# zabaras/deep-turbulence

Measured on AMD Instinct MI355X. Metric: flow-field samples/sec (fwd+log-det+bwd), 64x256x256x4; optimizer step: HipAdam (one-launch Adam, same update as torch.optim.Adam), higher is better.
Workload: dtype f32

## Files before the change

deep-turbulence_amd/csrc/tmg_common.h:

```cpp
#pragma once
#include <hip/hip_runtime.h>
#include <stdint.h>
#include <stdlib.h>
#include <atomic>

typedef float f32x4 __attribute__((ext_vector_type(4)));

__device__ __forceinline__ __amdgpu_buffer_rsrc_t tmg_make_rsrc(const void* base, unsigned bytes) {
    return __builtin_amdgcn_make_buffer_rsrc(const_cast<void*>(base), 0, (int)bytes, 0x00020000);
}
__device__ __forceinline__ float4 tmg_bload4(__amdgpu_buffer_rsrc_t rs, unsigned voff, unsigned soff) {
    const f32x4 v = __builtin_bit_cast(f32x4, __builtin_amdgcn_raw_buffer_load_b128(rs, (int)voff, (int)soff, 0));
    return make_float4(v[0], v[1], v[2], v[3]);
}

#define TMG_MAX_IN_SEG 3
#define TMG_MAX_OUT_SEG 3

struct TmgSeg {
    const float* p;
    int stride;
    int off;
    int n;
};
// ... 1 lines not shown
    float* p;
    int stride;
    int off;
    int n;
};

__device__ __forceinline__ float wave_sum(float v) {
#pragma unroll
    for (int o = 32; o > 0; o >>= 1) v += __shfl_xor(v, o, 64);
    return v;
}

__device__ __forceinline__ float block_sum_256(float v, float* red ) {
    v = wave_sum(v);
    const int lane = threadIdx.x & 63, w = threadIdx.x >> 6;
    __syncthreads();
    if (lane == 0) red[w] = v;
    __syncthreads();
    return red[0] + red[1] + red[2] + red[3];
}

__device__ __forceinline__ float out_scale_of(const float* kappa) {
    if (!kappa) return 1.0f;
    float k = *kappa;
    k = fminf(fmaxf(k, -4.0f), 1.3862943611198906f);
    return expf(k);
}

#define TMG_PICK_SEG(PTYPE_, ARR, C_, PTR_, STRIDE_, OFF_)                                                \
    PTYPE_ PTR_ = ARR[0].p;                                                                               \
    int STRIDE_ = ARR[0].stride, OFF_ = ARR[0].off;                                                       \
    if (C_ >= ARR[0].n) {                                                                                 \
        C_ -= ARR[0].n; PTR_ = ARR[1].p; STRIDE_ = ARR[1].stride; OFF_ = ARR[1].off;                      \
        if (C_ >= ARR[1].n) { C_ -= ARR[1].n; PTR_ = ARR[2].p; STRIDE_ = ARR[2].stride; OFF_ = ARR[2].off; } \
    }
#define TMG_PICK_OSEG(ARR, NL_, PTR_, STRIDE_, OFF_) TMG_PICK_SEG(float*, ARR, NL_, PTR_, STRIDE_, OFF_)

template <typename P>
__device__ __forceinline__ float4 load_in4(const P& p, int b, int iy, int ix, int c) {
    float4 v = make_float4(0.f, 0.f, 0.f, 0.f);
    if (p.pad_rep) {
        iy = min(max(iy, 0), p.Hin - 1);
        ix = min(max(ix, 0), p.Win - 1);
    } else if (iy < 0 || iy >= p.Hin || ix < 0 || ix >= p.Win) {
        return v;
    }
    if (c >= p.Cin) return v;
    const size_t pix = ((size_t)b * p.Hin + iy) * p.Win + ix;
    if (p.vec4) {
        int cl = c;
        TMG_PICK_SEG(const float*, p.in, cl, sp, ss, so)
        v = *reinterpret_cast<const float4*>(sp + pix * ss + so + cl);
    } else {
        float t[4];
#pragma unroll
        for (int e = 0; e < 4; ++e) {
            int cl = c + e;
            float x = 0.f;
            if (cl < p.Cin) {
                TMG_PICK_SEG(const float*, p.in, cl, sp, ss, so)
                x = sp[pix * ss + so + cl];
            }
            t[e] = x;
        }
        v = make_float4(t[0], t[1], t[2], t[3]);
    }
    if (p.in_scale) {
        float* f = reinterpret_cast<float*>(&v);
#pragma unroll
        for (int e = 0; e < 4; ++e)
            if (c + e < p.Cin) f[e] = f[e] * p.in_scale[c + e] + p.in_shift[c + e];
    }
    if (p.relu_in) {
        v.x = fmaxf(v.x, 0.f);
        v.y = fmaxf(v.y, 0.f);
        v.z = fmaxf(v.z, 0.f);
        v.w = fmaxf(v.w, 0.f);
    }
    return v;
}

template <int U = 8, typename P>
__device__ __forceinline__ void stage_patch(const P& p, float* lds, int b, int iy0, int ix0, int PH, int PW, int c0,
                                            int kch, int CS, int swz = 0) {
    const int k4 = kch >> 2;
    const int items = PH * PW * k4;
    const int nt = blockDim.x;
    const unsigned mk = k4 > 1 ? 0xFFFFFFFFu / (unsigned)k4 + 1u : 0u;
    const unsigned mp = 0xFFFFFFFFu / (unsigned)PW + 1u;
    for (int base = threadIdx.x; base < items; base += nt * U) {
        float4 v[U];
        int dst[U];
#pragma unroll
        for (int u = 0; u < U; ++u) {
            const int it = base + u * nt;
            dst[u] = -1;
            if (it < items) {
                const int pix = k4 > 1 ? (int)__umulhi((unsigned)it, mk) : it;
                const int c4 = it - pix * k4;
                const int py = (int)__umulhi((unsigned)pix, mp);
                const int px = pix - py * PW;
                v[u] = load_in4(p, b, iy0 + py, ix0 + px, c0 + 4 * c4);
                dst[u] = pix * CS + ((4 * c4) ^ ((px & 1) ? swz : 0));
            }
        }
#pragma unroll
        for (int u = 0; u < U; ++u)
            if (dst[u] >= 0) *reinterpret_cast<float4*>(lds + dst[u]) = v[u];
    }
}

static __device__ float tmg_zero_page[64];

#if defined(__HIP_DEVICE_COMPILE__)
#define TMG_PACKED_F32 __attribute__((target("packed-fp32-ops")))
#else
#define TMG_PACKED_F32
#endif

typedef float f32x2 __attribute__((ext_vector_type(2)));
#define TMG_GAS __attribute__((address_space(1)))
__device__ __forceinline__ float4 tmg_ldg4(const float* p) {
    const f32x4 v = *(const TMG_GAS f32x4*)p;
    return make_float4(v[0], v[1], v[2], v[3]);
}
__device__ __forceinline__ float2 tmg_ldg2(const float* p) {
    const f32x2 v = *(const TMG_GAS f32x2*)p;
    return make_float2(v[0], v[1]);
}
__device__ __forceinline__ float tmg_ldg1(const float* p) { return *(const TMG_GAS float*)p; }

__device__ __forceinline__ int tmg_xcd_block(int b, int G) {
    if (G < 16) return b;
    const int qn = G >> 3, rn = G & 7, x = b & 7;
    return x * qn + min(x, rn) + (b >> 3);
}
struct TmgTileRange { int first, end, step; };
__device__ __forceinline__ TmgTileRange tmg_xcd_tiles(int ntiles, int b, int G) {
    if (G < 16 || ntiles < 64) return TmgTileRange{b, ntiles, G};
    const int x = b & 7;
    const int nb = (G >> 3) + (x < (G & 7) ? 1 : 0);
    const int lo = (int)(((long long)ntiles * x) >> 3), hi = (int)(((long long)ntiles * (x + 1)) >> 3);
    return TmgTileRange{lo + (b >> 3), hi, nb};
}

template <typename P>
__device__ __forceinline__ const float* in4_addr(const P& p, int b, int iy, int ix, int c, bool& oob) {
    const int iyc = min(max(iy, 0), p.Hin - 1), ixc = min(max(ix, 0), p.Win - 1);
    oob = !p.pad_rep && (iy != iyc || ix != ixc);
    const size_t pix = ((size_t)b * p.Hin + iyc) * p.Win + ixc;
    int cl = c;
    TMG_PICK_SEG(const float*, p.in, cl, sp, ss, so)
    const float* a = sp + pix * ss + so + cl;
    return (oob || c >= p.Cin) ? tmg_zero_page : a;
}

template <int U = 4, typename P>
__device__ __forceinline__ void stage_patch_bf(const P& p, float* lds, int b, int iy0, int ix0, int PH, int PW, int c0,
                                               int kch, int CS) {
    if (!p.vec4) {
        stage_patch<U>(p, lds, b, iy0, ix0, PH, PW, c0, kch, CS);
        return;
    }
    const int k4 = kch >> 2;
    const int items = PH * PW * k4;
    const int nt = blockDim.x;
    const unsigned mk = k4 > 1 ? 0xFFFFFFFFu / (unsigned)k4 + 1u : 0u;
    const unsigned mp = 0xFFFFFFFFu / (unsigned)PW + 1u;
    for (int base = threadIdx.x; base < items; base += nt * U) {
        float4 v[U];
        const float* a[U];
        int dst[U];
        unsigned oobm = 0;
#pragma unroll
        for (int u = 0; u < U; ++u) {
            const int it = min(base + u * nt, items - 1);
            const int pix = k4 > 1 ? (int)__umulhi((unsigned)it, mk) : it;
            const int c4 = it - pix * k4;
            const int py = (int)__umulhi((unsigned)pix, mp);
            const int px = pix - py * PW;
            bool oob;
            a[u] = in4_addr(p, b, iy0 + py, ix0 + px, c0 + 4 * c4, oob);
            oobm |= (oob ? 1u : 0u) << u;
            dst[u] = (base + u * nt < items) ? pix * CS + 4 * c4 : -1;
        }
#pragma unroll
        for (int u = 0; u < U; ++u) v[u] = *reinterpret_cast<const float4*>(a[u]);
#pragma unroll
        for (int u = 0; u < U; ++u) {
            if (p.in_scale && !((oobm >> u) & 1u)) {
                const int it = min(base + u * nt, items - 1);
                const int pix = k4 > 1 ? (int)__umulhi((unsigned)it, mk) : it;
                const int c = c0 + 4 * (it - pix * k4);
                float* f = reinterpret_cast<float*>(&v[u]);
#pragma unroll
                for (int e = 0; e < 4; ++e)
                    if (c + e < p.Cin) f[e] = f[e] * p.in_scale[c + e] + p.in_shift[c + e];
            }
            if (p.relu_in) {
                v[u].x = fmaxf(v[u].x, 0.f); v[u].y = fmaxf(v[u].y, 0.f);
                v[u].z = fmaxf(v[u].z, 0.f); v[u].w = fmaxf(v[u].w, 0.f);
            }
            if (dst[u] >= 0) *reinterpret_cast<float4*>(lds + dst[u]) = v[u];
        }
    }
}

template <int U>
struct StageRegs {
    float4 v[U];
    int dst[U];
};

template <int U, typename P>
__device__ __forceinline__ void stage_issue(const P& p, StageRegs<U>& R, int b, int iy0, int ix0, int PH, int PW, int c0, int kch,
                                            int CS) {
    const int k4 = kch >> 2;
    const int items = PH * PW * k4;
    const int nt = blockDim.x;
    const unsigned mk = k4 > 1 ? 0xFFFFFFFFu / (unsigned)k4 + 1u : 0u;
    const unsigned mp = 0xFFFFFFFFu / (unsigned)PW + 1u;
#pragma unroll
    for (int u = 0; u < U; ++u) {
        const int it = threadIdx.x + u * nt;
        R.dst[u] = -1;
        if (it < items) {
            const int pix = k4 > 1 ? (int)__umulhi((unsigned)it, mk) : it;
            const int c4 = it - pix * k4;
            const int py = (int)__umulhi((unsigned)pix, mp);
            const int px = pix - py * PW;
            R.v[u] = load_in4(p, b, iy0 + py, ix0 + px, c0 + 4 * c4);
            R.dst[u] = pix * CS + 4 * c4;
        }
    }
}

template <int U, typename P>
__device__ __forceinline__ void stage_commit(const P& p, StageRegs<U>& R, float* lds, int b, int iy0, int ix0, int PH, int PW,
                                             int c0, int kch, int CS) {
#pragma unroll
    for (int u = 0; u < U; ++u)
        if (R.dst[u] >= 0) *reinterpret_cast<float4*>(lds + R.dst[u]) = R.v[u];
    const int k4 = kch >> 2;
    const int items = PH * PW * k4;
    const unsigned mk = k4 > 1 ? 0xFFFFFFFFu / (unsigned)k4 + 1u : 0u;
    const unsigned mp = 0xFFFFFFFFu / (unsigned)PW + 1u;
    for (int it = threadIdx.x + U * blockDim.x; it < items; it += blockDim.x) {
        const int pix = k4 > 1 ? (int)__umulhi((unsigned)it, mk) : it;
        const int c4 = it - pix * k4;
        const int py = (int)__umulhi((unsigned)pix, mp);
        const int px = pix - py * PW;
        *reinterpret_cast<float4*>(lds + pix * CS + 4 * c4) = load_in4(p, b, iy0 + py, ix0 + px, c0 + 4 * c4);
    }
}

static inline void tmg_lds_optin(const void* fn, std::atomic<uint64_t>& done) {
    int dev = 0;
    (void)hipGetDevice(&dev);
    const uint64_t bit = 1ull << (dev & 63);
    if (done.load(std::memory_order_relaxed) & bit) return;
    (void)hipFuncSetAttribute(fn, hipFuncAttributeMaxDynamicSharedMemorySize, 160 * 1024);
    done.fetch_or(bit, std::memory_order_relaxed);
}
#define TMG_LDS_OPTIN(FN)                                              \
    do {                                                               \
        static std::atomic<uint64_t> done__{0};                        \
        tmg_lds_optin(reinterpret_cast<const void*>(FN), done__);      \
// ... 62 lines not shown
```

deep-turbulence_amd/csrc/tmg_pointwise.hip:

```cpp
#include "tmg_common.h"
#include <stdlib.h>

#define LN5 1.6094379124341003f
#define LOG2PI 1.8378770664093453f

static inline int grid_for(size_t n, int cap = 4096) {
    size_t b = (n + 255) / 256;
    return (int)(b < (size_t)cap ? (b ? b : 1) : cap);
}

__global__ __launch_bounds__(256) void affine_apply_kernel(const float* __restrict__ hh, int hs, int ho, const float* x2, int xs,
                                                           int xo, float* y2, int ys, int yo, float* __restrict__ rsave,
                                                           float* __restrict__ logdet, int pix_per_img, int Ch, int reverse, int vec,
                                                           const float* x1, int x1s, float* y1, int y1s, int hpair) {
    __shared__ float red[4];
    const int b = blockIdx.y;
    const size_t base = (size_t)b * pix_per_img;
    const size_t total = (size_t)pix_per_img * Ch;
    float ld = 0.f;
    if (vec) {
        const int c4n = Ch >> 2;
        const size_t tot4 = (size_t)pix_per_img * c4n;
        for (size_t i = blockIdx.x * (size_t)256 + threadIdx.x; i < tot4; i += (size_t)gridDim.x * 256) {
            const size_t pix = base + i / c4n;
// ... 574 lines not shown
}

__global__ void bn_finalize_kernel(const float* __restrict__ sum, const float* __restrict__ csq, const float* __restrict__ gamma,
                                   const float* __restrict__ beta, float* __restrict__ rmean, float* __restrict__ rvar,
                                   float* __restrict__ out, int C, float n, float eps, float momentum) {
    const int c = blockIdx.x * blockDim.x + threadIdx.x;
    if (c >= C) return;
    const float mean = sum[c] / n, var = csq[c] / n;
    const float rstd = rsqrtf(var + eps);
    const float a = gamma[c] * rstd;
    out[c] = mean;
    out[C + c] = var;
    out[2 * C + c] = rstd;
    out[3 * C + c] = a;
    out[4 * C + c] = beta[c] - mean * a;
    if (rmean) {
        rmean[c] = rmean[c] * (1.f - momentum) + momentum * mean;
        rvar[c] = rvar[c] * (1.f - momentum) + momentum * var * (n / fmaxf(n - 1.f, 1.f));
    }
}

__global__ void bn_bwd_apply_kernel(const float* __restrict__ x, int xs, int xo, const float* __restrict__ g, int gs, int go,
                                    const float* __restrict__ a, const float* __restrict__ bsh, const float* __restrict__ mean,
                                    const float* __restrict__ rstd, const float* __restrict__ gamma, const float* __restrict__ m0,
                                    const float* __restrict__ m1, float* __restrict__ dx, int ds, int dof, size_t npix, int C,
                                    int accumulate, float m_scale) {
    const size_t total = npix * C;
    for (size_t i = blockIdx.x * (size_t)blockDim.x + threadIdx.x; i < total; i += (size_t)gridDim.x * blockDim.x) {
        const size_t pix = i / C;
        const int c = i % C;
        const float xv = x[pix * xs + xo + c];
        const float u = xv * a[c] + bsh[c];
        const float du = u > 0.f ? g[pix * gs + go + c] : 0.f;
        const float xh = (xv - mean[c]) * rstd[c];
        const float v = gamma[c] * rstd[c] * (du - m0[c] * m_scale - xh * m1[c] * m_scale);
        float* d = dx + pix * ds + dof + c;
        *d = accumulate ? (*d + v) : v;
    }
}

__global__ void masked_add_kernel(const float* __restrict__ src, int ss, int so, const float* __restrict__ ref, int rs_, int ro,
                                  const float* __restrict__ add, int as, int ao, float* dst, int ds, int dof, size_t npix, int n,
                                  int accumulate) {
    const size_t total = npix * n;
    for (size_t i = blockIdx.x * (size_t)blockDim.x + threadIdx.x; i < total; i += (size_t)gridDim.x * blockDim.x) {
        const size_t pix = i / n;
        const int c = i % n;
        float v = src ? src[pix * ss + so + c] : 0.f;
        if (ref && !(ref[pix * rs_ + ro + c] > 0.f)) v = 0.f;
        if (add) v += add[pix * as + ao + c];
        float* d = dst + pix * ds + dof + c;
        *d = accumulate ? (*d + v) : v;
    }
}

__global__ __launch_bounds__(256) void masked_add4_kernel(const float* __restrict__ src, int ss, int so, const float* __restrict__ ref, int rs_, int ro,
                                   const float* __restrict__ add, int as, int ao, float* dst, int ds, int dof, unsigned npix, int nq,
                                   int accumulate) {
    const unsigned total = npix * (unsigned)nq;
    for (unsigned i = blockIdx.x * blockDim.x + threadIdx.x; i < total; i += gridDim.x * blockDim.x) {
        const unsigned pix = i / (unsigned)nq;
        const unsigned c = 4u * (i - pix * (unsigned)nq);
        float4 v = src ? *reinterpret_cast<const float4*>(src + (size_t)pix * ss + so + c) : make_float4(0.f, 0.f, 0.f, 0.f);
        if (ref) {
            const float4 r = *reinterpret_cast<const float4*>(ref + (size_t)pix * rs_ + ro + c);
            if (!(r.x > 0.f)) v.x = 0.f;
            if (!(r.y > 0.f)) v.y = 0.f;
            if (!(r.z > 0.f)) v.z = 0.f;
            if (!(r.w > 0.f)) v.w = 0.f;
        }
        if (add) {
            const float4 a = *reinterpret_cast<const float4*>(add + (size_t)pix * as + ao + c);
            v.x += a.x; v.y += a.y; v.z += a.z; v.w += a.w;
        }
        float4* d = reinterpret_cast<float4*>(dst + (size_t)pix * ds + dof + c);
        if (accumulate) {
            const float4 o = *d;
            v.x += o.x; v.y += o.y; v.z += o.z; v.w += o.w;
        }
        *d = v;
    }
}

struct C1P {
    TmgSeg in[TMG_MAX_IN_SEG];
    int nseg, vec4;
    int B, Hin, Win;
    int Cin;
    const float* in_scale;
    const float* in_shift;
    int relu_in, pad_rep;
    const float* w;
    int w_rows, w_split, w_gap;
    const float* add; int add_stride, add_off;
    int fill4;
    float* out; int out_stride, out_off;
    int TW_log2, tiles_x, tiles_y, KCH;
};

__global__ __launch_bounds__(256) void c1_fwd_kernel(C1P p) {
    extern __shared__ __attribute__((aligned(16))) float lds[];
    const int tid = threadIdx.x;
    int t = blockIdx.x;
    const int tx = t % p.tiles_x;
    t /= p.tiles_x;
    const int ty = t % p.tiles_y;
    const int b = t / p.tiles_y;
    const int TWl = p.TW_log2, TW = 1 << TWl, TH = 256 >> TWl;
    const int PW = TW + 2, PH = TH + 2;
    const int oy0 = ty * TH, ox0 = tx * TW;
    const int row = tid >> TWl, col = tid & (TW - 1);
    const int Cpad = (p.Cin + 3) & ~3;
    float acc = 0.f;
    for (int c0 = 0; c0 < Cpad; c0 += p.KCH) {
        const int kch = min(p.KCH, Cpad - c0);
        const int CS = kch + 4;
        float* lw = lds + PH * PW * CS;
        __syncthreads();
        stage_patch_bf(p, lds, b, oy0 - 1, ox0 - 1, PH, PW, c0, kch, CS);
        for (int i = tid; i < 9 * kch; i += 256) {
            const int tap = i / kch, c = i - tap * kch;
            const int cs = c0 + c;
            lw[i] = (cs < p.w_rows) ? p.w[(size_t)(cs + (cs < p.w_split ? 0 : p.w_gap)) * 9 + tap] : 0.f;
        }
        __syncthreads();
#pragma unroll
        for (int tap = 0; tap < 9; ++tap) {
            const int tyy = tap / 3, txx = tap - tyy * 3;
            const float* pp = lds + ((row + tyy) * PW + col + txx) * CS;
            const float* wp = lw + tap * kch;
            for (int c = 0; c < kch; c += 4) {
                const float4 a = *reinterpret_cast<const float4*>(pp + c);
                const float4 w4 = *reinterpret_cast<const float4*>(wp + c);
                acc += a.x * w4.x + a.y * w4.y + a.z * w4.z + a.w * w4.w;
            }
        }
    }
    const int oy = oy0 + row, ox = ox0 + col;
    if (oy < p.Hin && ox < p.Win) {
        const size_t opx = ((size_t)b * p.Hin + oy) * p.Win + ox;
        if (p.add) acc += p.add[opx * p.add_stride + p.add_off];
        float* o = p.out + opx * p.out_stride + p.out_off;
        if (p.fill4) *reinterpret_cast<float4*>(o) = make_float4(acc, 0.f, 0.f, 0.f);
        else *o = acc;
    }
}

struct C1X2P {
    TmgSeg in[TMG_MAX_IN_SEG];
    int nseg, vec4;
    int B, Hin, Win;
    int Cin;
    const float* in_scale;
    const float* in_shift;
    int relu_in, pad_rep;
    const float* w1;
    const float* w2;
    int w_rows, w_split, w_gap, w2_d1;
    const float* add1; int a1_stride, a1_off;
    const float* add2; int a2_stride, a2_off;
    float* out; int out_stride;
    int TW_log2, tiles_x, tiles_y, KCH;
};

template <int CG>
__global__ __launch_bounds__(256) void c1x2_fwd_kernel(C1X2P p) {
    extern __shared__ __attribute__((aligned(16))) float lds[];
    constexpr int NPX = 256 / CG;
    const int tid = threadIdx.x;
    const int pid = tid / CG, cg = tid % CG;
    const bool lead = cg == 0;
    int t = tmg_xcd_block((int)blockIdx.x, (int)gridDim.x);
    const int tx = t % p.tiles_x;
    t /= p.tiles_x;
    const int ty = t % p.tiles_y;
    const int b = t / p.tiles_y;
    const int TWl = p.TW_log2, TW = 1 << TWl, TH = NPX >> TWl;
    const int PW = TW + 4, PH = TH + 4;
    const int RW = TW + 2, RH = TH + 2;
    const int oy0 = ty * TH, ox0 = tx * TW;
    const int row = pid >> TWl, col = pid & (TW - 1);
    const int Cpad = (p.Cin + 3) & ~3;
    int ry[2], rx[2];
    bool rok[2];
    ry[0] = row + 1; rx[0] = col + 1; rok[0] = true;
    const int nring = 2 * RW + 2 * (RH - 2);
    {
        rok[1] = pid < nring;
        int i = rok[1] ? pid : 0;
        if (i < RW) { ry[1] = 0; rx[1] = i; }
        else if (i < 2 * RW) { ry[1] = RH - 1; rx[1] = i - RW; }
        else if (i < 2 * RW + RH - 2) { ry[1] = 1 + i - 2 * RW; rx[1] = 0; }
        else { ry[1] = 1 + i - (2 * RW + RH - 2); rx[1] = RW - 1; }
    }
    const bool ring_wave = (tid & ~63) / CG < nring;
    const int oy = oy0 + row, ox = ox0 + col;
    const bool own = oy < p.Hin && ox < p.Win;
    const size_t opx = ((size_t)b * p.Hin + min(oy, p.Hin - 1)) * p.Win + min(ox, p.Win - 1);
    const float a2v = *((p.add2 && own && lead) ? p.add2 + opx * p.a2_stride + p.a2_off : tmg_zero_page);
    float a1v[2];
    bool rin[2];
#pragma unroll
    for (int u = 0; u < 2; ++u) {
        const int y = oy0 - 1 + ry[u], x = ox0 - 1 + rx[u];
        rin[u] = rok[u] && y >= 0 && y < p.Hin && x >= 0 && x < p.Win;
        const size_t px = ((size_t)b * p.Hin + min(max(y, 0), p.Hin - 1)) * p.Win + min(max(x, 0), p.Win - 1);
        a1v[u] = *((p.add1 && rin[u] && lead) ? p.add1 + px * p.a1_stride + p.a1_off : tmg_zero_page);
    }
    float acc1[2] = {0.f, 0.f}, acc2 = 0.f;
    for (int c0 = 0; c0 < Cpad; c0 += p.KCH) {
        const int kch = min(p.KCH, Cpad - c0);
        const int CS = kch + 4;
        float* lw1 = lds + PH * PW * CS;
        float* lw2 = lw1 + 9 * p.KCH;
        __syncthreads();
        stage_patch_bf(p, lds, b, oy0 - 2, ox0 - 2, PH, PW, c0, kch, CS);
        for (int i = tid; i < 9 * kch; i += 256) {
            const int tap = i / kch, c = i - tap * kch;
            const int cs = c0 + c;
            const bool ok = cs < p.w_rows;
            const size_t r = (size_t)(cs + (cs < p.w_split ? 0 : p.w_gap)) * 9 + tap;
            lw1[i] = ok ? p.w1[r] : 0.f;
            lw2[i] = ok ? p.w2[r] : 0.f;
        }
        __syncthreads();
#pragma unroll
        for (int tap = 0; tap < 9; ++tap) {
            const int tyy = tap / 3, txx = tap - tyy * 3;
            const float* w1p = lw1 + tap * kch;
            const float* w2p = lw2 + tap * kch;
            const float* p0 = lds + ((ry[0] + tyy) * PW + rx[0] + txx) * CS;
            const float* p1 = lds + ((ry[1] + tyy) * PW + rx[1] + txx) * CS;
            for (int c = 4 * cg; c < kch; c += 4 * CG) {
                const float4 wa = *reinterpret_cast<const float4*>(w1p + c);
                const float4 wb = *reinterpret_cast<const float4*>(w2p + c);
                const float4 x0 = *reinterpret_cast<const float4*>(p0 + c);
                acc1[0] += x0.x * wa.x + x0.y * wa.y + x0.z * wa.z + x0.w * wa.w;
                acc2 += x0.x * wb.x + x0.y * wb.y + x0.z * wb.z + x0.w * wb.w;
                if (ring_wave) {
                    const float4 x1 = *reinterpret_cast<const float4*>(p1 + c);
                    acc1[1] += x1.x * wa.x + x1.y * wa.y + x1.z * wa.z + x1.w * wa.w;
                }
            }
        }
    }
#pragma unroll
    for (int o = 1; o < CG; o <<= 1) {
        acc1[0] += __shfl_xor(acc1[0], o);
        acc1[1] += __shfl_xor(acc1[1], o);
        acc2 += __shfl_xor(acc2, o);
    }
    __syncthreads();
    float* ld1 = lds;
    if (lead) {
#pragma unroll
        for (int u = 0; u < 2; ++u)
            if (rok[u]) ld1[ry[u] * RW + rx[u]] = rin[u] ? fmaxf(acc1[u] + a1v[u], 0.f) : 0.f;
    }
    const float d1own = acc1[0] + a1v[0];
    __syncthreads();
    if (!lead) return;
    float w2d[9];
#pragma unroll
    for (int tap = 0; tap < 9; ++tap) w2d[tap] = p.w2[(size_t)p.w2_d1 * 9 + tap];
#pragma unroll
    for (int tap = 0; tap < 9; ++tap) {
        const int tyy = tap / 3, txx = tap - tyy * 3;
        acc2 += w2d[tap] * ld1[(row + tyy) * RW + col + txx];
    }
    if (own) *reinterpret_cast<float4*>(p.out + opx * p.out_stride) = make_float4(d1own, acc2 + a2v, 0.f, 0.f);
}

struct C1BP {
    TmgSeg in[TMG_MAX_IN_SEG];
    int nseg, vec4;
    int B, Hin, Win;
    int Cin;
    const float* in_scale;
    const float* in_shift;
    int relu_in, pad_rep;
    const float* w;
    float* dW;
    const float* dd; int dd_stride, dd_off;
    const float* dref; int dref_stride, dref_off;
    TmgOSeg g[TMG_MAX_OUT_SEG];
    int TW_log2, tiles_x, tiles_y, ntiles, KCH;
};

__global__ __launch_bounds__(256) void c1_bwd_kernel(C1BP p) {
    extern __shared__ __attribute__((aligned(16))) float lds[];
    const int tid = threadIdx.x;
    const int TWl = p.TW_log2, TW = 1 << TWl, TH = 256 >> TWl;
    const int PW = TW + 2, PH = TH + 2;
    const int row = tid >> TWl, col = tid & (TW - 1);
    const int Cpad = (p.Cin + 3) & ~3;
    const int nchunks = (Cpad + p.KCH - 1) / p.KCH;
    float* ldd = lds;
    float* lw = ldd + ((PH * PW + 3) & ~3);
    float* lin = lw + 9 * p.KCH;
    float wacc[2][8];
#pragma unroll
    for (int k = 0; k < 2; ++k)
#pragma unroll
        for (int c = 0; c < 8; ++c) wacc[k][c] = 0.f;

    for (int tile = blockIdx.x; tile < p.ntiles; tile += gridDim.x) {
        int t = tile;
        const int tx = t % p.tiles_x;
        t /= p.tiles_x;
        const int ty = t % p.tiles_y;
        const int b = t / p.tiles_y;
        const int oy0 = ty * TH, ox0 = tx * TW;
        __syncthreads();
        for (int i = tid; i < PH * PW; i += 256) {
            const int py = i / PW, px = i - py * PW;
            const int y = oy0 - 1 + py, x = ox0 - 1 + px;
            float v = 0.f;
            if (y >= 0 && y < p.Hin && x >= 0 && x < p.Win) {
                const size_t pix = ((size_t)b * p.Hin + y) * p.Win + x;
                v = p.dd[pix * p.dd_stride + p.dd_off];
                if (p.dref && !(p.dref[pix * p.dref_stride + p.dref_off] > 0.f)) v = 0.f;
            }
            ldd[i] = v;
        }
        __syncthreads();
        float dnb[9];
#pragma unroll
        for (int tap = 0; tap < 9; ++tap) {
            const int ky = tap / 3, kx = tap - ky * 3;
            dnb[tap] = ldd[(row + 2 - ky) * PW + col + 2 - kx];
        }
        const int oy = oy0 + row, ox = ox0 + col;
        const bool inside = oy < p.Hin && ox < p.Win;
        const size_t opix = ((size_t)b * p.Hin + oy) * p.Win + ox;
#pragma unroll
        for (int ch = 0; ch < 8; ++ch) {
            if (ch >= nchunks) break;
            const int c0 = ch * p.KCH;
            const int kch = min(p.KCH, Cpad - c0);
            const int CS = kch + 4;
            __syncthreads();
            stage_patch_bf(p, lin, b, oy0 - 1, ox0 - 1, PH, PW, c0, kch, CS);
            for (int i = tid; i < 9 * kch; i += 256) {
                const int tap = i / kch, c = i - tap * kch;
                lw[i] = (c0 + c < p.Cin) ? p.w[(size_t)(c0 + c) * 9 + tap] : 0.f;
            }
            __syncthreads();
            if (inside) {
                for (int c = 0; c < kch; ++c) {
                    const int ci = c0 + c;
                    if (ci >= p.Cin) break;
                    float v = 0.f;
#pragma unroll
// ... 676 lines not shown
}

extern "C" int tmg_bn_finalize(const void* sum, const void* csq, const void* gamma, const void* beta, void* rmean, void* rvar, void* out,
                               const int64_t* dims, const float* fl, hipStream_t st) {
    const int C = (int)dims[0];
    hipLaunchKernelGGL(bn_finalize_kernel, dim3((C + 255) / 256), dim3(256), 0, st, (const float*)sum, (const float*)csq, (const float*)gamma,
                       (const float*)beta, (float*)rmean, (float*)rvar, (float*)out, C, (float)dims[1], fl[0], fl[1]);
    TMG_CHECK_LAUNCH();
    return 0;
}

extern "C" int tmg_masked_add(const void* src, const int64_t* s_d, const void* ref, const int64_t* r_d, const void* add,
                              const int64_t* a_d, void* dst, const int64_t* d_d, const int64_t* dims, hipStream_t st) {
    const size_t npix = (size_t)dims[0];
    const int n = (int)dims[1];
    if (npix == 0 || n == 0) return 0;
    const TmgD2 sd = tmg_opt_d2(src, s_d), rd = tmg_opt_d2(ref, r_d), ad = tmg_opt_d2(add, a_d);
    {
        long long m = n | d_d[0] | d_d[1];
        uintptr_t al = (uintptr_t)dst;
        if (src) { m |= s_d[0] | s_d[1]; al |= (uintptr_t)src; }
        if (ref) { m |= r_d[0] | r_d[1]; al |= (uintptr_t)ref; }
        if (add) { m |= a_d[0] | a_d[1]; al |= (uintptr_t)add; }
        if ((m & 3) == 0 && (al & 15) == 0 && npix * (size_t)(n / 4) < (1ull << 31)) {
            hipLaunchKernelGGL(masked_add4_kernel, dim3(grid_for(npix * (n / 4))), dim3(256), 0, st, (const float*)src, sd.stride,
                               sd.off, (const float*)ref, rd.stride, rd.off, (const float*)add, ad.stride, ad.off, (float*)dst, (int)d_d[0],
                               (int)d_d[1], (unsigned)npix, n / 4, (int)dims[2]);
            TMG_CHECK_LAUNCH();
            return 0;
        }
    }
    hipLaunchKernelGGL(masked_add_kernel, dim3(grid_for(npix * n)), dim3(256), 0, st, (const float*)src, sd.stride,
                       sd.off, (const float*)ref, rd.stride, rd.off, (const float*)add, ad.stride, ad.off, (float*)dst, (int)d_d[0], (int)d_d[1],
                       npix, n, (int)dims[2]);
    TMG_CHECK_LAUNCH();
    return 0;
}

static int c1_tile(int W, int H, int* twl) {
    int l = 0;
    while ((1 << l) < W) ++l;
    if (l > 5) l = 5;
    if (l < 3) l = 3;
    *twl = l;
    (void)H;
    return 0;
}

static int c1x2_fwd_impl(const void* const* in_ptrs, const int64_t* in_desc, int64_t nseg, const void* w1, const void* w2,
                         const void* add1, const int64_t* add1_d, const void* add2, const int64_t* add2_d, void* out,
                         const int64_t* out_d, const int64_t* dims, hipStream_t st, int64_t* plan) {
    C1X2P p;
    p.nseg = (int)nseg;
    p.vec4 = tmg_decode_in(p.in, in_ptrs, in_desc, nseg).vec4;
    p.B = (int)dims[0]; p.Hin = (int)dims[1]; p.Win = (int)dims[2]; p.Cin = (int)dims[3]; p.relu_in = (int)dims[4];
    p.w_rows = (dims[5] > 0 && dims[5] < p.Cin) ? (int)dims[5] : p.Cin;
    p.w_split = dims[6] > 0 ? (int)dims[6] : 0x7fffffff; p.w_gap = (int)dims[7]; p.w2_d1 = (int)dims[8];
    if (p.Cin & 3) p.vec4 = 0;
    p.pad_rep = 0; p.in_scale = nullptr; p.in_shift = nullptr;
    p.w1 = (const float*)w1; p.w2 = (const float*)w2;
    const TmgD2 a1 = tmg_opt_d2(add1, add1_d), a2 = tmg_opt_d2(add2, add2_d);
    p.add1 = (const float*)add1; p.a1_stride = a1.stride; p.a1_off = a1.off;
    p.add2 = (const float*)add2; p.a2_stride = a2.stride; p.a2_off = a2.off;
    if ((out_d[0] & 3) || out_d[1] != 0 || (((uintptr_t)out) & 15)) return -2;
    p.out = (float*)out; p.out_stride = (int)out_d[0];
    c1_tile(p.Win, p.Hin, &p.TW_log2);
    int CG = 1;
    long t256;
    {
        const int tw = 1 << p.TW_log2, th = 256 >> p.TW_log2;
        t256 = (long)p.B * ((p.Win + tw - 1) / tw) * ((p.Hin + th - 1) / th);
        const int Cq = (p.Cin + 3) / 4;
        if (t256 < 512 && Cq >= 4) CG = 4;
        else if (t256 < 1024 && Cq >= 2) CG = 2;
    }
    const int NPX = 256 / CG;
    while ((NPX >> p.TW_log2) < 4 && p.TW_log2 > 3) --p.TW_log2;
    const int TW = 1 << p.TW_log2, TH = NPX >> p.TW_log2;
    if (2 * (TW + 2) + 2 * TH > NPX) return -2;
    p.tiles_x = (p.Win + TW - 1) / TW;
    p.tiles_y = (p.Hin + TH - 1) / TH;
    const int Cpad = (p.Cin + 3) & ~3;
    p.KCH = Cpad < 32 ? Cpad : 32;
    size_t lds_floats = (size_t)(TH + 4) * (TW + 4) * (p.KCH + 4) + 18 * p.KCH;
    const size_t d1_floats = 2 * (size_t)(((TH + 2) * (TW + 2) + 3) & ~3);
    if (lds_floats < d1_floats) lds_floats = d1_floats;
    if (plan) {
        const int64_t v[12] = {CG, p.TW_log2, TH, p.tiles_x, p.tiles_y, t256, p.KCH, (Cpad + p.KCH - 1) / p.KCH, 2 * (TW + 2) + 2 * TH,
                               (int64_t)p.B * p.tiles_x * p.tiles_y, (int64_t)(lds_floats * 4), p.vec4};
        for (int i = 0; i < 12; ++i) plan[i] = v[i];
        return 0;
    }
    TmgProf prof(TMG_PROF_C1X2, 4.0 * p.B * (double)p.Hin * p.Win * (p.Cin + 4 + (p.add1 ? 1 : 0) + (p.add2 ? 1 : 0)), st);
    const dim3 grid(p.B * p.tiles_x * p.tiles_y);
    if (CG == 1) {
        TMG_LDS_OPTIN((&c1x2_fwd_kernel<1>));
        hipLaunchKernelGGL(c1x2_fwd_kernel<1>, grid, dim3(256), lds_floats * 4, st, p);
    } else if (CG == 2) {
        TMG_LDS_OPTIN((&c1x2_fwd_kernel<2>));
        hipLaunchKernelGGL(c1x2_fwd_kernel<2>, grid, dim3(256), lds_floats * 4, st, p);
    } else {
        TMG_LDS_OPTIN((&c1x2_fwd_kernel<4>));
        hipLaunchKernelGGL(c1x2_fwd_kernel<4>, grid, dim3(256), lds_floats * 4, st, p);
    }
    TMG_CHECK_LAUNCH();
    return 0;
}

extern "C" int tmg_c1x2_fwd(const void* const* in_ptrs, const int64_t* in_desc, int64_t nseg, const void* w1, const void* w2,
                            const void* add1, const int64_t* add1_d, const void* add2, const int64_t* add2_d, void* out,
                            const int64_t* out_d, const int64_t* dims, hipStream_t st) {
    return c1x2_fwd_impl(in_ptrs, in_desc, nseg, w1, w2, add1, add1_d, add2, add2_d, out, out_d, dims, st, nullptr);
}

extern "C" int tmg_c1x2_fwd_plan(const void* const* in_ptrs, const int64_t* in_desc, int64_t nseg, const void* w1, const void* w2,
                                 const void* add1, const int64_t* add1_d, const void* add2, const int64_t* add2_d, void* out,
                                 const int64_t* out_d, const int64_t* dims, hipStream_t st, int64_t* plan) {
    if (!plan) return -1;
    for (int i = 0; i < 12; ++i) plan[i] = -1;
    return c1x2_fwd_impl(in_ptrs, in_desc, nseg, w1, w2, add1, add1_d, add2, add2_d, out, out_d, dims, st, plan);
}

static int c1_fwd_impl(const void* const* in_ptrs, const int64_t* in_desc, int64_t nseg, const void* w, const void* add,
                       const int64_t* add_d, void* out, const int64_t* out_d, const int64_t* dims, hipStream_t st, int64_t* plan) {
    C1P p;
    p.nseg = (int)nseg;
    p.vec4 = tmg_decode_in(p.in, in_ptrs, in_desc, nseg).vec4;
    p.B = (int)dims[0]; p.Hin = (int)dims[1]; p.Win = (int)dims[2]; p.Cin = (int)dims[3]; p.relu_in = (int)dims[4];
    p.w_rows = (dims[5] > 0 && dims[5] < p.Cin) ? (int)dims[5] : p.Cin;
    p.fill4 = (int)dims[6];
    p.w_split = dims[7] > 0 ? (int)dims[7] : 0x7fffffff; p.w_gap = (int)dims[8];
    const TmgD2 ad = tmg_opt_d2(add, add_d);
    p.add = (const float*)add; p.add_stride = ad.stride; p.add_off = ad.off;
    if (p.Cin & 3) p.vec4 = 0;
    p.pad_rep = 0; p.in_scale = nullptr; p.in_shift = nullptr;
    p.w = (const float*)w; p.out = (float*)out; p.out_stride = (int)out_d[0]; p.out_off = (int)out_d[1];
    c1_tile(p.Win, p.Hin, &p.TW_log2);
    const int TW = 1 << p.TW_log2, TH = 256 >> p.TW_log2;
    p.tiles_x = (p.Win + TW - 1) / TW;
    p.tiles_y = (p.Hin + TH - 1) / TH;
    const int Cpad = (p.Cin + 3) & ~3;
    p.KCH = Cpad < 32 ? Cpad : 32;
    const size_t lds_bytes = ((size_t)(TH + 2) * (TW + 2) * (p.KCH + 4) + 9 * p.KCH) * 4;
    if (plan) {
        const int64_t v[9] = {p.TW_log2, TH, p.tiles_x, p.tiles_y, p.KCH, (Cpad + p.KCH - 1) / p.KCH, (int64_t)p.B * p.tiles_x * p.tiles_y,
                              (int64_t)lds_bytes, p.vec4};
        for (int i = 0; i < 9; ++i) plan[i] = v[i];
        return 0;
    }
    TMG_LDS_OPTIN((&c1_fwd_kernel));
    hipLaunchKernelGGL(c1_fwd_kernel, dim3(p.B * p.tiles_x * p.tiles_y), dim3(256), lds_bytes, st, p);
    TMG_CHECK_LAUNCH();
    return 0;
}

extern "C" int tmg_c1_fwd_add(const void* const* in_ptrs, const int64_t* in_desc, int64_t nseg, const void* w, const void* add,
                              const int64_t* add_d, void* out, const int64_t* out_d, const int64_t* dims, hipStream_t st) {
    return c1_fwd_impl(in_ptrs, in_desc, nseg, w, add, add_d, out, out_d, dims, st, nullptr);
}

extern "C" int tmg_c1_fwd(const void* const* in_ptrs, const int64_t* in_desc, int64_t nseg, const void* w, void* out,
                          const int64_t* out_d, const int64_t* dims, hipStream_t st) {
    return c1_fwd_impl(in_ptrs, in_desc, nseg, w, nullptr, nullptr, out, out_d, dims, st, nullptr);
}

extern "C" int tmg_c1_fwd_plan(const void* const* in_ptrs, const int64_t* in_desc, int64_t nseg, const void* w, const void* add,
                               const int64_t* add_d, void* out, const int64_t* out_d, const int64_t* dims, hipStream_t st, int64_t* plan) {
    if (!plan) return -1;
    for (int i = 0; i < 9; ++i) plan[i] = -1;
    return c1_fwd_impl(in_ptrs, in_desc, nseg, w, add, add_d, out, out_d, dims, st, plan);
}

extern "C" int tmg_c1_bwd(const void* const* in_ptrs, const int64_t* in_desc, int64_t nseg, const void* w, void* dW, const void* dd,
                          const int64_t* dd_d, const void* dref, const int64_t* dref_d, void* const* g_ptrs, const int64_t* g_desc,
                          int64_t ng, const int64_t* dims, hipStream_t st) {
    C1BP p;
    p.nseg = (int)nseg;
    p.vec4 = tmg_decode_in(p.in, in_ptrs, in_desc, nseg).vec4;
    p.B = (int)dims[0]; p.Hin = (int)dims[1]; p.Win = (int)dims[2]; p.Cin = (int)dims[3]; p.relu_in = (int)dims[4];
    if (p.Cin & 3) p.vec4 = 0;
    p.pad_rep = 0; p.in_scale = nullptr; p.in_shift = nullptr;
    p.w = (const float*)w; p.dW = (float*)dW;
    p.dd = (const float*)dd; p.dd_stride = (int)dd_d[0]; p.dd_off = (int)dd_d[1];
    const TmgD2 rd = tmg_opt_d2(dref, dref_d);
    p.dref = (const float*)dref; p.dref_stride = rd.stride; p.dref_off = rd.off;
    tmg_decode_out(p.g, g_ptrs, g_desc, ng);
    c1_tile(p.Win, p.Hin, &p.TW_log2);
    const int TW = 1 << p.TW_log2, TH = 256 >> p.TW_log2;
    p.tiles_x = (p.Win + TW - 1) / TW;
    p.tiles_y = (p.Hin + TH - 1) / TH;
    p.ntiles = p.B * p.tiles_x * p.tiles_y;
    const int Cpad = (p.Cin + 3) & ~3;
    p.KCH = Cpad < 32 ? Cpad : 32;
    if ((Cpad + p.KCH - 1) / p.KCH > 8) return -2;
    const int PP = (TH + 2) * (TW + 2);
    const size_t lds_bytes = ((size_t)((PP + 3) & ~3) + 9 * p.KCH + (size_t)PP * (p.KCH + 4)) * 4;
    TMG_LDS_OPTIN((&c1_bwd_kernel));
    int gx = p.ntiles < 1024 ? p.ntiles : 1024;
    hipLaunchKernelGGL(c1_bwd_kernel, dim3(gx), dim3(256), lds_bytes, st, p);
    TMG_CHECK_LAUNCH();
    return 0;
}

extern "C" int tmg_dense2_bwd(const void* const* in_ptrs, const int64_t* in_desc, int64_t nseg, const void* w1, const void* w2,
                              void* dW1, void* dW2, const void* GD, int64_t gd_stride, const void* Dp, int64_t d_stride,
                              const void* const* g0_ptrs, const int64_t* g0_desc, void* const* out_ptrs, const int64_t* out_desc,
                              int64_t ng, const void* add0, int64_t add0_stride, const int64_t* dims, hipStream_t st) {
    D2BP p;
    p.nseg = (int)nseg;
    p.vec4 = tmg_decode_in(p.in, in_ptrs, in_desc, nseg).vec4;
    p.B = (int)dims[0]; p.Hin = (int)dims[1]; p.Win = (int)dims[2]; p.Cin = (int)dims[3]; p.cin_nn = (int)dims[4];
    p.rows1 = (int)dims[5]; p.rows2 = (int)dims[6];
    p.relu_in = 1; p.pad_rep = 0; p.in_scale = nullptr; p.in_shift = nullptr;
    if (p.Cin & 3) p.vec4 = 0;
    p.w1 = (const float*)w1; p.w2 = (const float*)w2; p.dW1 = (float*)dW1; p.dW2 = (float*)dW2;
    p.GD = (const float*)GD; p.gd_stride = (int)gd_stride; p.Dp = (const float*)Dp; p.d_stride = (int)d_stride;
    if (!tmg_decode_in(p.g0, g0_ptrs, g0_desc, ng, 2).vec4) p.vec4 = 0;
    tmg_decode_out(p.out, out_ptrs, out_desc, ng, 2);
    for (int i = 0; i < 2; ++i)
        if (((p.out[i].stride | p.out[i].off) & 3) || (((uintptr_t)p.out[i].p) & 15)) p.vec4 = 0;
    p.add0 = (const float*)add0; p.add0_stride = (int)add0_stride;
    p.dd1_out = (float*)dims[7]; p.dd2_out = (float*)dims[8]; p.dd_stride = (int)dims[9];
    p.dd_quad = dims[12] && p.dd1_out && p.dd2_out == p.dd1_out + 1 && !(p.dd_stride & 3) && !(((uintptr_t)p.dd1_out) & 15);
    if (dims[12] && !p.dd_quad) return -4;
    p.g0_masked = dims[13] != 0;
    if (p.g0_masked && (add0 || p.cin_nn > 16 || p.dW1 || p.dW2 || (p.gd_stride & 3) || (((uintptr_t)p.GD) & 15))) return -4;
// ... 441 lines not shown
```

Before: 1507.

## Register-block 3x3 single-output convs into 4-pixel strips with padded LDS rows

The c1 and c1x2 forward kernels now have each thread compute a strip of four adjacent output pixels. The six loaded input vectors are reused across the three horizontal taps, and channel work is split among QS lanes with a shuffle reduction at the end, using packed f32x2 FMAs. LDS rows get per-row padding to avoid bank conflicts. The c1x2 ring of halo pixels is handled by dedicated wave groups doing horizontal and vertical strips. This cuts LDS loads per FMA, at the cost of more complex indexing and tighter tile constraints that can make the planner reject some shapes.

```diff
diff --git a/deep-turbulence_amd/csrc/tmg_common.h b/deep-turbulence_amd/csrc/tmg_common.h
--- a/deep-turbulence_amd/csrc/tmg_common.h
+++ b/deep-turbulence_amd/csrc/tmg_common.h
@@ -107,7 +107,7 @@
 
 template <int U = 8, typename P>
 __device__ __forceinline__ void stage_patch(const P& p, float* lds, int b, int iy0, int ix0, int PH, int PW, int c0,
-                                            int kch, int CS, int swz = 0) {
+                                            int kch, int CS, int swz = 0, int row_pad = 0) {
     const int k4 = kch >> 2;
     const int items = PH * PW * k4;
     const int nt = blockDim.x;
@@ -126,7 +126,7 @@
                 const int py = (int)__umulhi((unsigned)pix, mp);
                 const int px = pix - py * PW;
                 v[u] = load_in4(p, b, iy0 + py, ix0 + px, c0 + 4 * c4);
-                dst[u] = pix * CS + ((4 * c4) ^ ((px & 1) ? swz : 0));
+                dst[u] = pix * CS + py * row_pad + ((4 * c4) ^ ((px & 1) ? swz : 0));
             }
         }
 #pragma unroll
@@ -182,9 +182,9 @@
 
 template <int U = 4, typename P>
 __device__ __forceinline__ void stage_patch_bf(const P& p, float* lds, int b, int iy0, int ix0, int PH, int PW, int c0,
-                                               int kch, int CS) {
+                                               int kch, int CS, int row_pad = 0) {
     if (!p.vec4) {
-        stage_patch<U>(p, lds, b, iy0, ix0, PH, PW, c0, kch, CS);
+        stage_patch<U>(p, lds, b, iy0, ix0, PH, PW, c0, kch, CS, 0, row_pad);
         return;
     }
     const int k4 = kch >> 2;
@@ -207,7 +207,7 @@
             bool oob;
             a[u] = in4_addr(p, b, iy0 + py, ix0 + px, c0 + 4 * c4, oob);
             oobm |= (oob ? 1u : 0u) << u;
-            dst[u] = (base + u * nt < items) ? pix * CS + 4 * c4 : -1;
+            dst[u] = (base + u * nt < items) ? pix * CS + py * row_pad + 4 * c4 : -1;
         }
 #pragma unroll
         for (int u = 0; u < U; ++u) v[u] = *reinterpret_cast<const float4*>(a[u]);
diff --git a/deep-turbulence_amd/csrc/tmg_pointwise.hip b/deep-turbulence_amd/csrc/tmg_pointwise.hip
--- a/deep-turbulence_amd/csrc/tmg_pointwise.hip
+++ b/deep-turbulence_amd/csrc/tmg_pointwise.hip
@@ -680,6 +680,62 @@
     }
 }
 
+template <bool TWO>
+__device__ __forceinline__ void c1_strip_line(const float* a, int sa, const float* w1, const float* w2, int wt, f32x2 (&s1)[4], f32x2 (&s2)[4]) {
+    f32x4 x[6];
+#pragma unroll
+    for (int j = 0; j < 6; ++j) x[j] = *reinterpret_cast<const f32x4*>(a + j * sa);
+#pragma unroll
+    for (int t = 0; t < 3; ++t) {
+        const f32x4 wa = *reinterpret_cast<const f32x4*>(w1 + t * wt);
+#pragma unroll
+        for (int i = 0; i < 4; ++i) {
+            s1[i] = __builtin_elementwise_fma(x[i + t].lo, wa.lo, s1[i]);
+            s1[i] = __builtin_elementwise_fma(x[i + t].hi, wa.hi, s1[i]);
+        }
+        if (TWO) {
+            const f32x4 wb = *reinterpret_cast<const f32x4*>(w2 + t * wt);
+#pragma unroll
+            for (int i = 0; i < 4; ++i) {
+                s2[i] = __builtin_elementwise_fma(x[i + t].lo, wb.lo, s2[i]);
+                s2[i] = __builtin_elementwise_fma(x[i + t].hi, wb.hi, s2[i]);
+            }
+        }
+    }
+}
+
+template <bool TWO, bool VERT, int KCH>
+__device__ __forceinline__ void c1_strip_chunk(int kch_rt, const float* a, int RP, const float* w1, const float* w2, int c_first, int c_step,
+                                               f32x2 (&s1)[4], f32x2 (&s2)[4]) {
+    const int kch = KCH ? KCH : kch_rt, CS = kch + 4;
+    const int la = VERT ? CS : RP, sa = VERT ? RP : CS, wl = VERT ? kch : 3 * kch, wt = VERT ? 3 * kch : kch;
+    for (int c = c_first; c < kch; c += c_step) {
+        if (KCH) {
+#pragma unroll
+            for (int l = 0; l < 3; ++l) c1_strip_line<TWO>(a + c + l * la, sa, w1 + c + l * wl, w2 + c + l * wl, wt, s1, s2);
+        } else {
+#pragma unroll 1
+            for (int l = 0; l < 3; ++l) c1_strip_line<TWO>(a + c + l * la, sa, w1 + c + l * wl, w2 + c + l * wl, wt, s1, s2);
+        }
+    }
+}
+
+template <bool TWO, bool VERT, int KMIN>
+__device__ __forceinline__ void c1_strip_any(int kch, const float* a, int RP, const float* w1, const float* w2, int c_first, int c_step,
+                                             f32x2 (&s1)[4], f32x2 (&s2)[4]) {
+    if (KMIN <= 8 && kch == 8) c1_strip_chunk<TWO, VERT, 8>(kch, a, RP, w1, w2, c_first, c_step, s1, s2);
+    else if (KMIN <= 16 && kch == 16) c1_strip_chunk<TWO, VERT, 16>(kch, a, RP, w1, w2, c_first, c_step, s1, s2);
+    else if (kch == 32) c1_strip_chunk<TWO, VERT, 32>(kch, a, RP, w1, w2, c_first, c_step, s1, s2);
+    else c1_strip_chunk<TWO, VERT, 0>(kch, a, RP, w1, w2, c_first, c_step, s1, s2);
+}
+
+__host__ __device__ inline int c1_row_pad(int PW, int CS, int QS) {
+    const int R = PW * (CS >> 2);
+    return QS >= 4 ? 4 * ((16 - (R & 15)) & 15) : 4 * ((2 - (R & 3)) & 3);
+}
+
+__host__ __device__ inline int c1_fwd_qs_log2(int KCH) { return KCH >= 16 ? 2 : (KCH >= 8 ? 1 : 0); }
+
 struct C1P {
     TmgSeg in[TMG_MAX_IN_SEG];
     int nseg, vec4;
@@ -696,7 +752,7 @@
     int TW_log2, tiles_x, tiles_y, KCH;
 };
 
-__global__ __launch_bounds__(256) void c1_fwd_kernel(C1P p) {
+__global__ __launch_bounds__(256, 4) void c1_fwd_kernel(C1P p) {
     extern __shared__ __attribute__((aligned(16))) float lds[];
     const int tid = threadIdx.x;
     int t = blockIdx.x;
@@ -707,40 +763,52 @@
     const int TWl = p.TW_log2, TW = 1 << TWl, TH = 256 >> TWl;
     const int PW = TW + 2, PH = TH + 2;
     const int oy0 = ty * TH, ox0 = tx * TW;
-    const int row = tid >> TWl, col = tid & (TW - 1);
+    const int QSl = c1_fwd_qs_log2(p.KCH), QS = 1 << QSl;
+    const int item = tid >> QSl, q = tid & (QS - 1);
+    const bool active = item < 64;
+    const int row = (item & 63) >> (TWl - 2), col = 4 * (item & ((TW >> 2) - 1));
     const int Cpad = (p.Cin + 3) & ~3;
-    float acc = 0.f;
+    const int oy = oy0 + row, ox = ox0 + col;
+    const size_t opx = ((size_t)b * p.Hin + min(oy, p.Hin - 1)) * p.Win;
+    bool mine[4];
+    float av[4];
+#pragma unroll
+    for (int i = 0; i < 4; ++i) {
+        mine[i] = active && q == 0 && oy < p.Hin && ox + i < p.Win;
+        av[i] = *((p.add && mine[i]) ? p.add + (opx + ox + i) * p.add_stride + p.add_off : tmg_zero_page);
+    }
+    f32x2 acc[4] = {};
     for (int c0 = 0; c0 < Cpad; c0 += p.KCH) {
         const int kch = min(p.KCH, Cpad - c0);
         const int CS = kch + 4;
-        float* lw = lds + PH * PW * CS;
+        const int pad = c1_row_pad(PW, CS, QS), RP = PW * CS + pad;
+        float* lw = lds + PH * RP;
         __syncthreads();
-        stage_patch_bf(p, lds, b, oy0 - 1, ox0 - 1, PH, PW, c0, kch, CS);
+        stage_patch_bf(p, lds, b, oy0 - 1, ox0 - 1, PH, PW, c0, kch, CS, pad);
         for (int i = tid; i < 9 * kch; i += 256) {
             const int tap = i / kch, c = i - tap * kch;
             const int cs = c0 + c;
             lw[i] = (cs < p.w_rows) ? p.w[(size_t)(cs + (cs < p.w_split ? 0 : p.w_gap)) * 9 + tap] : 0.f;
         }
         __syncthreads();
-#pragma unroll
-        for (int tap = 0; tap < 9; ++tap) {
-            const int tyy = tap / 3, txx = tap - tyy * 3;
-            const float* pp = lds + ((row + tyy) * PW + col + txx) * CS;
-            const float* wp = lw + tap * kch;
-            for (int c = 0; c < kch; c += 4) {
-                const float4 a = *reinterpret_cast<const float4*>(pp + c);
-                const float4 w4 = *reinterpret_cast<const float4*>(wp + c);
-                acc += a.x * w4.x + a.y * w4.y + a.z * w4.z + a.w * w4.w;
-            }
-        }
-    }
-    const int oy = oy0 + row, ox = ox0 + col;
-    if (oy < p.Hin && ox < p.Win) {
-        const size_t opx = ((size_t)b * p.Hin + oy) * p.Win + ox;
-        if (p.add) acc += p.add[opx * p.add_stride + p.add_off];
-        float* o = p.out + opx * p.out_stride + p.out_off;
-        if (p.fill4) *reinterpret_cast<float4*>(o) = make_float4(acc, 0.f, 0.f, 0.f);
-        else *o = acc;
+        if (active) {
+            const float* a = lds + row * RP + col * CS;
+            c1_strip_any<false, false, 8>(kch, a, RP, lw, lw, 4 * q, 4 * QS, acc, acc);
+        }
+    }
+    float r[4];
+#pragma unroll
+    for (int i = 0; i < 4; ++i) r[i] = acc[i].x + acc[i].y;
+    for (int o = 1; o < QS; o <<= 1) {
+#pragma unroll
+        for (int i = 0; i < 4; ++i) r[i] += __shfl_xor(r[i], o);
+    }
+#pragma unroll
+    for (int i = 0; i < 4; ++i) {
+        if (!mine[i]) continue;
+        float* o = p.out + (opx + ox + i) * p.out_stride + p.out_off;
+        if (p.fill4) *reinterpret_cast<float4*>(o) = make_float4(r[i] + av[i], 0.f, 0.f, 0.f);
+        else *o = r[i] + av[i];
     }
 }
 
@@ -762,12 +830,14 @@
 };
 
 template <int CG>
-__global__ __launch_bounds__(256) void c1x2_fwd_kernel(C1X2P p) {
+__global__ __launch_bounds__(256, CG == 4 ? 3 : 4) void c1x2_fwd_kernel(C1X2P p) {
     extern __shared__ __attribute__((aligned(16))) float lds[];
-    constexpr int NPX = 256 / CG;
-    const int tid = threadIdx.x;
-    const int pid = tid / CG, cg = tid % CG;
-    const bool lead = cg == 0;
+    constexpr int NPX = 256 / CG, QS = 2 * CG, KMIN = CG == 4 ? 32 : 8;
+    const int tid = threadIdx.x, lane = tid & 63;
+    const bool own_w = tid < 128, vert = tid >= 192;
+    const int q = QS > 4 ? (lane & 3) | ((lane >> 5) << 2) : (lane & (QS - 1));
+    const int item = (tid >= 64 && own_w ? 64 / QS : 0) + (QS > 4 ? (lane & 31) >> 2 : lane / QS);
+    const bool lead = q == 0;
     int t = tmg_xcd_block((int)blockIdx.x, (int)gridDim.x);
     const int tx = t % p.tiles_x;
     t /= p.tiles_x;
@@ -777,42 +847,31 @@
     const int PW = TW + 4, PH = TH + 4;
     const int RW = TW + 2, RH = TH + 2;
     const int oy0 = ty * TH, ox0 = tx * TW;
-    const int row = pid >> TWl, col = pid & (TW - 1);
     const int Cpad = (p.Cin + 3) & ~3;
-    int ry[2], rx[2];
-    bool rok[2];
-    ry[0] = row + 1; rx[0] = col + 1; rok[0] = true;
-    const int nring = 2 * RW + 2 * (RH - 2);
-    {
-        rok[1] = pid < nring;
-        int i = rok[1] ? pid : 0;
-        if (i < RW) { ry[1] = 0; rx[1] = i; }
-        else if (i < 2 * RW) { ry[1] = RH - 1; rx[1] = i - RW; }
-        else if (i < 2 * RW + RH - 2) { ry[1] = 1 + i - 2 * RW; rx[1] = 0; }
-        else { ry[1] = 1 + i - (2 * RW + RH - 2); rx[1] = RW - 1; }
-    }
-    const bool ring_wave = (tid & ~63) / CG < nring;
-    const int oy = oy0 + row, ox = ox0 + col;
-    const bool own = oy < p.Hin && ox < p.Win;
-    const size_t opx = ((size_t)b * p.Hin + min(oy, p.Hin - 1)) * p.Win + min(ox, p.Win - 1);
-    const float a2v = *((p.add2 && own && lead) ? p.add2 + opx * p.a2_stride + p.a2_off : tmg_zero_page);
-    float a1v[2];
-    bool rin[2];
-#pragma unroll
-    for (int u = 0; u < 2; ++u) {
-        const int y = oy0 - 1 + ry[u], x = ox0 - 1 + rx[u];
-        rin[u] = rok[u] && y >= 0 && y < p.Hin && x >= 0 && x < p.Win;
-        const size_t px = ((size_t)b * p.Hin + min(max(y, 0), p.Hin - 1)) * p.Win + min(max(x, 0), p.Win - 1);
-        a1v[u] = *((p.add1 && rin[u] && lead) ? p.add1 + px * p.a1_stride + p.a1_off : tmg_zero_page);
-    }
-    float acc1[2] = {0.f, 0.f}, acc2 = 0.f;
+    const int SPRl = TWl - 2, SPR = 1 << SPRl;
+    const int NV = (TH >> 2) + 1;
+    int ry0, rx0;
+    bool active = true;
+    if (own_w) {
+        ry0 = (item >> SPRl) + 1; rx0 = 4 * (item & (SPR - 1)) + 1;
+    } else if (!vert) {
+        active = item < 2 * SPR;
+        const int k = min(item, 2 * SPR - 1);
+        ry0 = k < SPR ? 0 : RH - 1; rx0 = 4 * (k & (SPR - 1)) + 1;
+    } else {
+        active = item < 2 * NV;
+        const int k = min(item, 2 * NV - 1), side = k >= NV ? 1 : 0;
+        ry0 = min(4 * (k - side * NV), RH - 4); rx0 = side ? RW - 1 : 0;
+    }
+    f32x2 h1[4] = {}, h2[4] = {};
     for (int c0 = 0; c0 < Cpad; c0 += p.KCH) {
         const int kch = min(p.KCH, Cpad - c0);
         const int CS = kch + 4;
-        float* lw1 = lds + PH * PW * CS;
+        const int pad = c1_row_pad(PW, CS, QS), RP = PW * CS + pad;
+        float* lw1 = lds + PH * RP;
         float* lw2 = lw1 + 9 * p.KCH;
         __syncthreads();
-        stage_patch_bf(p, lds, b, oy0 - 2, ox0 - 2, PH, PW, c0, kch, CS);
+        stage_patch_bf(p, lds, b, oy0 - 2, ox0 - 2, PH, PW, c0, kch, CS, pad);
         for (int i = tid; i < 9 * kch; i += 256) {
             const int tap = i / kch, c = i - tap * kch;
             const int cs = c0 + c;
@@ -822,51 +881,64 @@
             lw2[i] = ok ? p.w2[r] : 0.f;
         }
         __syncthreads();
-#pragma unroll
-        for (int tap = 0; tap < 9; ++tap) {
-            const int tyy = tap / 3, txx = tap - tyy * 3;
-            const float* w1p = lw1 + tap * kch;
-            const float* w2p = lw2 + tap * kch;
-            const float* p0 = lds + ((ry[0] + tyy) * PW + rx[0] + txx) * CS;
-            const float* p1 = lds + ((ry[1] + tyy) * PW + rx[1] + txx) * CS;
-            for (int c = 4 * cg; c < kch; c += 4 * CG) {
-                const float4 wa = *reinterpret_cast<const float4*>(w1p + c);
-                const float4 wb = *reinterpret_cast<const float4*>(w2p + c);
-                const float4 x0 = *reinterpret_cast<const float4*>(p0 + c);
-                acc1[0] += x0.x * wa.x + x0.y * wa.y + x0.z * wa.z + x0.w * wa.w;
-                acc2 += x0.x * wb.x + x0.y * wb.y + x0.z * wb.z + x0.w * wb.w;
-                if (ring_wave) {
-                    const float4 x1 = *reinterpret_cast<const float4*>(p1 + c);
-                    acc1[1] += x1.x * wa.x + x1.y * wa.y + x1.z * wa.z + x1.w * wa.w;
-                }
-            }
-        }
-    }
-#pragma unroll
-    for (int o = 1; o < CG; o <<= 1) {
-        acc1[0] += __shfl_xor(acc1[0], o);
-        acc1[1] += __shfl_xor(acc1[1], o);
-        acc2 += __shfl_xor(acc2, o);
+        if (active) {
+            const float* a = lds + ry0 * RP + rx0 * CS;
+            if (own_w) c1_strip_any<true, false, KMIN>(kch, a, RP, lw1, lw2, 4 * q, 4 * QS, h1, h2);
+            else if (!vert) c1_strip_any<false, false, KMIN>(kch, a, RP, lw1, lw1, 4 * q, 4 * QS, h1, h1);
+            else c1_strip_any<false, true, KMIN>(kch, a, RP, lw1, lw1, 4 * q, 4 * QS, h1, h1);
+        }
+    }
+    float s1[4], s2[4];
+#pragma unroll
+    for (int i = 0; i < 4; ++i) { s1[i] = h1[i].x + h1[i].y; s2[i] = h2[i].x + h2[i].y; }
+    const int y0 = oy0 - 1 + ry0, x0 = ox0 - 1 + rx0;
+    const long px0 = ((long)b * p.Hin + y0) * p.Win + x0, dpx = vert ? p.Win : 1;
+    float a1v[4], a2v[4];
+    bool rin[4];
+#pragma unroll
+    for (int i = 0; i < 4; ++i) {
+        const int y = y0 + (vert ? i : 0), x = x0 + (vert ? 0 : i);
+        rin[i] = active && y >= 0 && y < p.Hin && x >= 0 && x < p.Win;
+        const size_t px = (size_t)(rin[i] ? px0 + i * dpx : 0);
+        a1v[i] = *((p.add1 && rin[i] && lead) ? p.add1 + px * p.a1_stride + p.a1_off : tmg_zero_page);
+        a2v[i] = *((p.add2 && rin[i] && lead && own_w) ? p.add2 + px * p.a2_stride + p.a2_off : tmg_zero_page);
+    }
+#pragma unroll
+    for (int o = 1; o < QS; o <<= 1) {
+        const int m = o < 4 ? o : 32;
+#pragma unroll
+        for (int i = 0; i < 4; ++i) {
+            s1[i] += __shfl_xor(s1[i], m);
+            if (own_w) s2[i] += __shfl_xor(s2[i], m);
+        }
     }
     __syncthreads();
     float* ld1 = lds;
-    if (lead) {
-#pragma unroll
-        for (int u = 0; u < 2; ++u)
-            if (rok[u]) ld1[ry[u] * RW + rx[u]] = rin[u] ? fmaxf(acc1[u] + a1v[u], 0.f) : 0.f;
-    }
-    const float d1own = acc1[0] + a1v[0];
+    if (lead && active) {
+#pragma unroll
+        for (int i = 0; i < 4; ++i) {
+            s1[i] += a1v[i];
+            ld1[(ry0 + (vert ? i : 0)) * RW + rx0 + (vert ? 0 : i)] = rin[i] ? fmaxf(s1[i], 0.f) : 0.f;
+        }
+    }
     __syncthreads();
-    if (!lead) return;
+    if (!(lead && own_w)) return;
     float w2d[9];
 #pragma unroll
     for (int tap = 0; tap < 9; ++tap) w2d[tap] = p.w2[(size_t)p.w2_d1 * 9 + tap];
 #pragma unroll
-    for (int tap = 0; tap < 9; ++tap) {
-        const int tyy = tap / 3, txx = tap - tyy * 3;
-        acc2 += w2d[tap] * ld1[(row + tyy) * RW + col + txx];
-    }
-    if (own) *reinterpret_cast<float4*>(p.out + opx * p.out_stride) = make_float4(d1own, acc2 + a2v, 0.f, 0.f);
+    for (int l = 0; l < 3; ++l) {
+        const float2* rp = reinterpret_cast<const float2*>(ld1 + (ry0 - 1 + l) * RW + rx0 - 1);
+        const float2 r01 = rp[0], r23 = rp[1], r45 = rp[2];
+        const float r[6] = {r01.x, r01.y, r23.x, r23.y, r45.x, r45.y};
+#pragma unroll
+        for (int t = 0; t < 3; ++t)
+#pragma unroll
+            for (int i = 0; i < 4; ++i) s2[i] = fmaf(w2d[l * 3 + t], r[i + t], s2[i]);
+    }
+#pragma unroll
+    for (int i = 0; i < 4; ++i)
+        if (rin[i]) *reinterpret_cast<float4*>(p.out + (size_t)(px0 + i) * p.out_stride) = make_float4(s1[i], s2[i] + a2v[i], 0.f, 0.f);
 }
 
 struct C1BP {
@@ -1709,7 +1781,11 @@
     p.tiles_y = (p.Hin + TH - 1) / TH;
     const int Cpad = (p.Cin + 3) & ~3;
     p.KCH = Cpad < 32 ? Cpad : 32;
-    size_t lds_floats = (size_t)(TH + 4) * (TW + 4) * (p.KCH + 4) + 18 * p.KCH;
+    const int QS = 2 * CG;
+    if ((TH & 3) || (2 * (TW / 4) + 2 * (TH / 4 + 1)) * QS > 128) return -2;
+    const int klast = Cpad % p.KCH ? Cpad % p.KCH : p.KCH;
+    const int pitch = std::max((TW + 4) * (p.KCH + 4) + c1_row_pad(TW + 4, p.KCH + 4, QS), (TW + 4) * (klast + 4) + c1_row_pad(TW + 4, klast + 4, QS));
+    size_t lds_floats = (size_t)(TH + 4) * pitch + 18 * p.KCH;
     const size_t d1_floats = 2 * (size_t)(((TH + 2) * (TW + 2) + 3) & ~3);
     if (lds_floats < d1_floats) lds_floats = d1_floats;
     if (plan) {
@@ -1768,7 +1844,10 @@
     p.tiles_y = (p.Hin + TH - 1) / TH;
     const int Cpad = (p.Cin + 3) & ~3;
     p.KCH = Cpad < 32 ? Cpad : 32;
-    const size_t lds_bytes = ((size_t)(TH + 2) * (TW + 2) * (p.KCH + 4) + 9 * p.KCH) * 4;
+    const int QS = 1 << c1_fwd_qs_log2(p.KCH);
+    const int klast = Cpad % p.KCH ? Cpad % p.KCH : p.KCH;
+    const int pitch = std::max((TW + 2) * (p.KCH + 4) + c1_row_pad(TW + 2, p.KCH + 4, QS), (TW + 2) * (klast + 4) + c1_row_pad(TW + 2, klast + 4, QS));
+    const size_t lds_bytes = ((size_t)(TH + 2) * pitch + 9 * p.KCH) * 4;
     if (plan) {
         const int64_t v[9] = {p.TW_log2, TH, p.tiles_x, p.tiles_y, p.KCH, (Cpad + p.KCH - 1) / p.KCH, (int64_t)p.B * p.tiles_x * p.tiles_y,
                               (int64_t)lds_bytes, p.vec4};
```

Result: slower. 1487 (-1.3%).
